# jibo27/3DGS_Hierarchical_Training

Hardware: AMD Instinct MI355X
Metric: train-step images/sec + fwd+bwd ms @1M Gaussians, 980x545; 1/2/4/8 GPU (higher is better)
Workload: dtype f32

## Files before the change

### 3dgs_hierarchical_training_amd/csrc/gsr_kernels.hip

```cpp
#include <hip/hip_runtime.h>
#include <hip/hip_ext.h>
#include <type_traits>
#include <stdint.h>
#include <stdio.h>
#include <string.h>

#include <algorithm>
#include <atomic>
#include <chrono>
#include <cmath>
#include <map>
#include <mutex>
#include <tuple>
#include <vector>

#include "../../include/gsr.h"
#include "gsr_math.h"
#include "adam_math.h"
#include "radix_sort.h"
#include "blend_common.h"

#ifndef GSR_K9_UNROLL
#define GSR_K9_UNROLL 2
#endif
// ... 1080 lines not shown
        for (int g = 0; g < kDbMaxGroups; g++) v[g] = g < db.G ? db.GT[(size_t)g * db.Tp + t] : 0u;
#pragma unroll
        for (int g = 0; g < kDbMaxGroups; g++) {
            if (g < db.G) db.GT[(size_t)g * db.Tp + t] = tot;
            tot += v[g];
        }
    }
    if (t >= db.T) tot = 0u;
    const uint32_t inc = wave_inclusive_sum(tot);
    if (lane == 63) s_w[wave] = inc;
    __syncthreads();
    lo = s_lo[0] + s_lo[1] + s_lo[2] + s_lo[3];
    all = s_all[0] + s_all[1] + s_all[2] + s_all[3];
    uint32_t add = 0u;
#pragma unroll
    for (int w = 0; w < 4; w++) add += w < wave ? s_w[w] : 0u;
    const uint32_t base_t = (uint32_t)min(lo + add + inc - tot, 0xffffffffull);
    if (t < db.T) db.tbase[t] = base_t;
    if (cut.key) {
        if (t < db.T) {
            const uint32_t e = cut.cur[0] < (uint32_t)kVcEntries ? cut.cur[0] : 0u;
            const bool use = cut.cur[9] != 0u && cut.owner_n[e] == (uint32_t)db.N;
            uint32_t ck = (uint32_t)(db.NC - 1);
            const uint32_t k = use ? cut.key[(size_t)e * db.T + t] : kCutOpenKey;
            if (k != kCutOpenKey && k != 0u) {
                const float d = __uint_as_float(k);
                const uint32_t kc = __float_as_uint(fmaf(d, cut.margin, d));
                int a = 0, b = db.NC;
                while (a < b) { const int m = (a + b) >> 1; if (s_bkey[m] <= kc) a = m + 1; else b = m; }
                ck = (uint32_t)max(a - 1, 0);
            }
            cut.chunk[t] = (uint16_t)ck;
            cut.flag[t] = 0u;
            if (use) atomicAdd(&cut.hist[ck], 1u);
            if (t == 0) cut.ctl[3] = use ? 1u : 0u;
        }
    }
    if (slab == 0 && tid == 0) {
        db.tbase[db.T] = (uint32_t)min(all, 0xffffffffull);
        *total_out = all;
        if (host_out) {
            __atomic_store_n(host_out + 2, (unsigned long long)g_onesweep_giveups, __ATOMIC_RELAXED);
            __atomic_store_n(host_out + 3, (unsigned long long)(window_overflow ? *window_overflow : 0u), __ATOMIC_RELAXED);
            __atomic_store_n(host_out, all, __ATOMIC_RELAXED);
            __threadfence_system();
            __atomic_store_n(host_out + 1, host_seq, __ATOMIC_RELAXED);
            __threadfence_system();
        }
        if (late_out) scan_report_late(late_out, all, host_seq);
    }
}

constexpr int kDbPairs = 1024;
__device__ __forceinline__ void lds_order() { __builtin_amdgcn_fence(__ATOMIC_ACQ_REL, "wavefront"); __builtin_amdgcn_wave_barrier(); }

__device__ __forceinline__ uint32_t cut_frame(const ListCut& cut, const int NC, uint32_t& deep)
{
    const int lane = threadIdx.x & 63;
    deep = 0u;
    if (cut.ctl[3] == 0u) return (uint32_t)(NC - 1);
    constexpr int kR = 32;
    uint32_t v[kR];
#pragma unroll
    for (int q = 0; q < kR; q++) { const int c = NC - 1 - 64 * q - lane; v[q] = (64 * q < NC && c >= 0) ? cut.hist[c] : 0u; }
    uint32_t acc = 0u;
#pragma unroll
    for (int q = 0; q < kR; q++) {
        if (64 * q >= NC) break;
        const int c = NC - 1 - 64 * q - lane;
        const uint32_t inc = acc + wave_inclusive_sum(v[q]);
        const unsigned long long over = __ballot(c >= 0 && inc > (uint32_t)cut.dmax);
        if (over) {
            const int l = (int)__builtin_ctzll(over);
            deep = (uint32_t)__builtin_amdgcn_readlane((int)(inc - v[q]), l);
            return (uint32_t)(NC - 1 - 64 * q - l);
        }
        acc = (uint32_t)__builtin_amdgcn_readlane((int)inc, 63);
    }
    for (int top = NC - 1 - 64 * kR; top >= 0; top -= 64) {
        const int c = top - lane;
        const uint32_t w = c >= 0 ? cut.hist[c] : 0u;
        const uint32_t inc = acc + wave_inclusive_sum(w);
        const unsigned long long over = __ballot(c >= 0 && inc > (uint32_t)cut.dmax);
        if (over) {
            const int l = (int)__builtin_ctzll(over);
            deep = (uint32_t)__builtin_amdgcn_readlane((int)(inc - w), l);
            return (uint32_t)(top - l);
        }
        acc = (uint32_t)__builtin_amdgcn_readlane((int)inc, 63);
    }
    deep = acc;
    return 0u;
}

template <typename Want>
__device__ __forceinline__ void cut_chunk_tiles(const DirectBin& db, const int c, const int W, const int H, const int tiles_x, const int tiles_y,
                                                const uint32_t* __restrict__ sorted_gid, const TileRec* __restrict__ sorted_rec,
                                                const Splat* __restrict__ splat, uint32_t* __restrict__ list, const uint32_t cap,
                                                uint32_t* s_txy , uint32_t* s_pos , Want&& want)
{
    const int lane = threadIdx.x & 63;
    const unsigned long long lt = lanemask_lt();
    const int j0 = c * db.S, j1 = min(db.N, j0 + db.S);
    const uint32_t* gt = db.GT + (size_t)(c / db.Cg) * db.Tp;
    const uint16_t* mr = db.M + (size_t)c * db.Tp;
    auto load_rec = [&](int j) -> TileRec { TileRec r; r.mask = 0u; r.rect = 1u << 24; if (j < j1) r = sorted_rec[j]; return r; };
// ... 22 lines not shown
        }
        if (nt == 0) break;
        lds_order();
        TileRec rA = load_rec(j0 + lane), rB = load_rec(j0 + 64 + lane);
        uint32_t gA = load_gid(j0 + lane), gB = load_gid(j0 + 64 + lane);
        for (int j = j0; j < j1; j += 64) {
            const TileRec r = rA;
            const uint32_t g = gA;
            rA = rB; gA = gB;
            rB = load_rec(j + 128 + lane);
            gB = load_gid(j + 128 + lane);
            const bool big = (r.rect & kTileRecBig) != 0u && r.mask != 0u;
            const uint32_t ww = (r.rect >> 24) & 63u, rx0 = r.rect & 0xfffu, ry0 = (r.rect >> 12) & 0xfffu;
            TileTest tt = {};
            int bx0 = 0, by0 = 0, bx1 = 0, by1 = 0;
            if (big) {
                const Splat sp = splat[g];
                tile_rect_tight(sp.px, sp.py, sp.radius, sp.ca, sp.cb, sp.cc, sp.op, W, H, tiles_x, tiles_y, bx0, by0, bx1, by1);
                tt = make_tile_test(sp.px, sp.py, sp.ca, sp.cb, sp.cc, sp.op);
            }
            const bool any_big = __ballot(big) != 0ull;
            for (int k = 0; k < nt; k++) {
                const uint32_t txy = s_txy[k], tx = txy & 0xffffu, ty = txy >> 16;
                const uint32_t dx = tx - rx0, dy = ty - ry0, bit = dy * ww + dx;
                bool in = !big && dx < ww && bit < 32u && ((r.mask >> bit) & 1u) != 0u;
                if (any_big && big) in = (int)tx >= bx0 && (int)tx < bx1 && (int)ty >= by0 && (int)ty < by1 && tile_accept(tt, (int)tx, (int)ty, W, H);
                const unsigned long long b = __ballot(in);
                if (b == 0ull) continue;
                const uint32_t p0 = s_pos[k];
                if (in) { const uint32_t pos = p0 + (uint32_t)__popcll(b & lt); if (pos < cap) list[pos] = g; }
                lds_order();
                if (lane == 0) s_pos[k] = p0 + (uint32_t)__popcll(b);
                lds_order();
            }
        }
        lds_order();
    }
}

#ifdef GSR_DB_TIMING
__device__ unsigned long long g_db_dbg[16];
#define DB_T(k) do { const unsigned long long now_ = __builtin_readcyclecounter(); if (lane == 0) dbt[k] += now_ - dbt_last; dbt_last = now_; } while (0)
#else
#define DB_T(k) do { } while (0)
#endif
template <bool PAIRS = false, int CUT = 0>
__global__ __launch_bounds__(64) void k_chunk_scatter(DirectBin db, int W, int H, int tiles_x, int tiles_y,
                                                      const uint32_t* __restrict__ sorted_gid, const TileRec* __restrict__ sorted_rec,
                                                      const Splat* __restrict__ splat, uint32_t* __restrict__ list, uint2* __restrict__ ranges,
                                                      uint32_t cap, const uint32_t* __restrict__ dkey = nullptr, uint2* __restrict__ pairs = nullptr,
                                                      ListCut cut = ListCut{})
{
    static_assert(!CUT || !PAIRS, "the list cut serves the plain direct binning");
    extern __shared__ unsigned long long s_dyn[];
    const int LT = db.Tp;
    unsigned long long* const s_mask = s_dyn;
    uint32_t* const s_cnt = reinterpret_cast<uint32_t*>(s_dyn + LT);
    uint32_t* const s_pair = s_cnt + LT;
    const int lane = threadIdx.x, b = (int)blockIdx.x;
    if (CUT == 2 && cut.ctl[2] == 0u) return;
    uint32_t cstar = 0u, ndeep = 0u;
    if (CUT == 1) cstar = cut_frame(cut, db.NC, ndeep);
    if (CUT == 2) cstar = cut.ctl[0];
    {
        const int t = b * 64 + lane;
        if (t < db.T) {
            uint32_t tend = db.tbase[t + 1];
            if (CUT == 1) {
                const uint32_t c1 = max((uint32_t)cut.chunk[t], cstar) + 1u;
                if (c1 < (uint32_t)db.NC) tend = db.tbase[t] + db.GT[(size_t)(c1 / (uint32_t)db.Cg) * db.Tp + t] + (uint32_t)db.M[(size_t)c1 * db.Tp + t];
                cut.tend[t] = tend;
            }
            const uint32_t lo = min(db.tbase[t], cap), hi = min(tend, cap);
            if (CUT != 2 || cut.flag[t]) ranges[t] = hi > lo ? make_uint2(lo, hi) : make_uint2(0u, 0u);
            if (CUT == 1) {
                const uint32_t e = cut.cur[0] < (uint32_t)kVcEntries ? cut.cur[0] : 0u;
                cut.key[(size_t)e * db.T + t] = 0u;
            }
        }
        if (CUT && b == 0 && lane == 0) {
            if (CUT == 1) {
                const uint32_t e = cut.cur[0] < (uint32_t)kVcEntries ? cut.cur[0] : 0u;
                cut.owner_n[e] = (uint32_t)db.N;
                cut.ctl[0] = cstar; cut.ctl[1] = ndeep;
                cut.stats[0] += 1u;
                cut.stats[3] += (uint32_t)(db.NC - 1) - min(cstar, (uint32_t)(db.NC - 1));
                cut.stats[4] += ndeep;
            } else { cut.stats[1] += 1u; cut.stats[2] += cut.ctl[2]; }
        }
    }
    const int per = (db.NC + 7) >> 3, kk = b >> 3, c = (b & 7) * per + kk;
    if (kk >= per || c >= db.NC) return;
    if (CUT && (uint32_t)c > cstar) {
        if (CUT == 1 && ndeep == 0u) return;
        uint32_t* const s_tile = s_pair;
        uint32_t* const s_pos = s_pair + 64;
        if (CUT == 1) cut_chunk_tiles(db, c, W, H, tiles_x, tiles_y, sorted_gid, sorted_rec, splat, list, cap, s_tile, s_pos,
                                      [&](uint32_t t) { return (uint32_t)cut.chunk[t] >= (uint32_t)c; });
        else cut_chunk_tiles(db, c, W, H, tiles_x, tiles_y, sorted_gid, sorted_rec, splat, list, cap, s_tile, s_pos,
                             [&](uint32_t t) { return cut.flag[t] != 0u && (uint32_t)cut.chunk[t] < (uint32_t)c; });
        return;
    }
    if (CUT == 2) return;
#ifdef GSR_DB_TIMING
    unsigned long long dbt[8] = {0, 0, 0, 0, 0, 0, 0, 0}, dbt_last = __builtin_readcyclecounter();
#endif
    {
        const uint32_t* gt = db.GT + (size_t)(c / db.Cg) * db.Tp;
        const uint16_t* mr = db.M + (size_t)c * db.Tp;
        constexpr int kRows = 36;
        for (int i0 = 0; i0 < LT; i0 += 64 * kRows) {
            uint32_t tb[kRows], gb[kRows], mc[kRows];
#pragma unroll
            for (int q = 0; q < kRows; q++) {
                const int i = i0 + 64 * q + lane;
                const bool v = i < LT && (uint32_t)i < (uint32_t)LT;
                tb[q] = v && i < db.T ? db.tbase[i] : 0u;
                gb[q] = v ? gt[i] : 0u;
                mc[q] = v ? (uint32_t)mr[i] : 0u;
            }
#pragma unroll
            for (int q = 0; q < kRows; q++) {
                const int i = i0 + 64 * q + lane;
                if (i < LT) { s_cnt[i] = tb[q] + gb[q] + mc[q]; s_mask[i] = 0ull; }
            }
        }
    }
    lds_order();
    DB_T(0);
    const unsigned long long me = 1ull << lane, lt = lanemask_lt();
    const int j0 = c * db.S, j1 = min(db.N, j0 + db.S);
    auto load_gid = [&](int j) -> uint32_t { return j < j1 ? (PAIRS ? (uint32_t)j : sorted_gid[j]) : 0u; };
    auto load_rec = [&](int j) -> TileRec { TileRec r; r.mask = 0u; r.rect = 1u << 24; if (j < j1) r = sorted_rec[j]; return r; };
    auto load_key = [&](int j) -> uint32_t { return (PAIRS && j < j1) ? dkey[j] : 0u; };
    uint32_t gA = load_gid(j0 + lane), gB = load_gid(j0 + 64 + lane);
    TileRec rA = load_rec(j0 + lane), rB = load_rec(j0 + 64 + lane);
    uint32_t kA = load_key(j0 + lane), kB = load_key(j0 + 64 + lane);
    for (int j = j0 + lane; j - lane < j1; j += 64) {
        const uint32_t g = gA;
        TileRec r = rA;
        const uint32_t kd = kA;
        gA = gB; rA = rB; kA = kB;
        gB = load_gid(j + 128);
        rB = load_rec(j + 128);
        kB = load_key(j + 128);
        const bool big = (r.rect & kTileRecBig) != 0u && r.mask != 0u, huge = big && r.mask > (uint32_t)kDbPairs;
        const unsigned long long bigs = __ballot(big && !huge), huges = __ballot(huge);
        const uint32_t cnt = huge ? 0u : tilerec_count(r);
        const uint32_t incl = wave_inclusive_sum(cnt);
        auto run_end = [&](int lo, uint32_t before) -> int {
            const unsigned long long over = __ballot(incl - before > (uint32_t)kDbPairs) & ~((1ull << lo) - 1ull);
            return over ? (int)__builtin_ctzll(over) : 64;
        };
        auto owners = [&](int lo, int hi, uint32_t before, bool with_or) {
            const bool mine = lane >= lo && lane < hi;
            if (!big && (with_or || mine)) {
                uint32_t* o = s_pair + (incl - cnt - before);
                small_rect_tiles(r, tiles_x, [&](uint32_t t) {
                    if (with_or) atomicOr(&s_mask[t], me);
                    if (mine) *o++ = (t << 6) | (uint32_t)lane;
                });
            }
            for (unsigned long long bm = bigs; bm != 0ull; bm &= bm - 1ull) {
                const int bl = (int)__builtin_ctzll(bm);
                const bool in_run = bl >= lo && bl < hi;
                if (!with_or && !in_run) continue;
                const uint32_t gg = (uint32_t)__builtin_amdgcn_readlane((int)g, bl), rect = (uint32_t)__builtin_amdgcn_readlane((int)r.rect, bl);
                uint32_t o = (uint32_t)__builtin_amdgcn_readlane((int)(incl - cnt), bl) - before;
                const Splat s = splat[gg];
                big_rect_tiles(s, rect, W, H, tiles_x, tiles_y, lane, [&](bool ok, uint32_t t) {
                    const unsigned long long acc = __ballot(ok);
                    if (ok) {
                        if (with_or) atomicOr(&s_mask[t], 1ull << bl);
                        if (in_run) s_pair[(o + (uint32_t)__popcll(acc & lt)) & (uint32_t)(kDbPairs - 1)] = (t << 6) | (uint32_t)bl;
                    }
                    o += (uint32_t)__popcll(acc);
                });
            }
        };
        int lo = 0, hi = run_end(0, 0u);
        uint32_t before = 0u;
        const bool one_run = hi == 64;
        DB_T(1);
        owners(0, hi, 0u, true);
        DB_T(2);
        for (unsigned long long bm = huges; bm != 0ull; bm &= bm - 1ull) {
            const int bl = (int)__builtin_ctzll(bm);
            const uint32_t gg = (uint32_t)__builtin_amdgcn_readlane((int)g, bl), rect = (uint32_t)__builtin_amdgcn_readlane((int)r.rect, bl);
            const Splat s = splat[gg];
            big_rect_tiles(s, rect, W, H, tiles_x, tiles_y, lane, [&](bool ok, uint32_t t) { if (ok && t < (uint32_t)db.T) atomicOr(&s_mask[t], 1ull << bl); });
        }
        asm volatile("" : "+v"(gA), "+v"(rA.mask), "+v"(rA.rect));
        if (PAIRS) asm volatile("" : "+v"(kA));
        lds_order();
        DB_T(3);
        for (;;) {
            const uint32_t P = (uint32_t)__builtin_amdgcn_readlane((int)incl, hi - 1) - before;
            for (uint32_t p0 = 0u; p0 < P; p0 += 512u) {
                const uint32_t left = P - p0;
                auto batch = [&](auto rounds_tag) {
                    constexpr int RN = decltype(rounds_tag)::value;
                    uint32_t e[RN], go[RN], base[RN], ko[PAIRS ? RN : 1];
                    unsigned long long mk[RN];
#pragma unroll
                    for (int q = 0; q < RN; q++) e[q] = s_pair[(p0 + 64u * q + (uint32_t)lane) & (uint32_t)(kDbPairs - 1)];
#pragma unroll
                    for (int q = 0; q < RN; q++) {
                        const bool v = 64u * q + (uint32_t)lane < left;
                        e[q] = v ? e[q] : 0xffffffffu;
                        const uint32_t t = v ? e[q] >> 6 : 0u;
                        go[q] = (uint32_t)__builtin_amdgcn_ds_bpermute((int)((e[q] & 63u) << 2), (int)g);
                        if (PAIRS) ko[q] = (uint32_t)__builtin_amdgcn_ds_bpermute((int)((e[q] & 63u) << 2), (int)kd);
                        mk[q] = s_mask[t];
                        base[q] = s_cnt[t];
                    }
#pragma unroll
                    for (int q = 0; q < RN; q++)
                        if (e[q] != 0xffffffffu) {
                            const uint32_t pos = base[q] + (uint32_t)__popcll(mk[q] & ((1ull << (e[q] & 63u)) - 1ull));
                            if (pos < cap) {
                                if (PAIRS) pairs[pos] = make_uint2(ko[q], go[q]);
                                else list[pos] = go[q];
                            }
                        }
                };
                if (left <= 128u) batch(std::integral_constant<int, 2>{});
                else if (left <= 256u) batch(std::integral_constant<int, 4>{});
                else if (left <= 384u) batch(std::integral_constant<int, 6>{});
                else batch(std::integral_constant<int, 8>{});
            }
            if (hi == 64) break;
            lds_order();
            before += P;
            lo = hi;
            hi = run_end(lo, before);
            owners(lo, hi, before, false);
            lds_order();
        }
        for (unsigned long long bm = huges; bm != 0ull; bm &= bm - 1ull) {
            const int bl = (int)__builtin_ctzll(bm);
            const uint32_t gg = (uint32_t)__builtin_amdgcn_readlane((int)g, bl), rect = (uint32_t)__builtin_amdgcn_readlane((int)r.rect, bl);
            const Splat s = splat[gg];
            big_rect_tiles(s, rect, W, H, tiles_x, tiles_y, lane, [&](bool ok, uint32_t t) {
                if (ok && t < (uint32_t)db.T) {
                    const uint32_t pos = s_cnt[t] + (uint32_t)__popcll(s_mask[t] & ((1ull << bl) - 1ull));
                    if (pos < cap) {
                        if (PAIRS) pairs[pos] = make_uint2((uint32_t)__builtin_amdgcn_readlane((int)kd, bl), gg);
                        else list[pos] = gg;
                    }
                }
            });
        }
        lds_order();
        DB_T(4);
        if (one_run) {
            const uint32_t P = (uint32_t)__builtin_amdgcn_readlane((int)incl, 63);
            for (uint32_t p0 = 0u; p0 < P; p0 += 512u) {
                const uint32_t left = P - p0;
                auto batch = [&](auto rounds_tag) {
                    constexpr int RN = decltype(rounds_tag)::value;
                    uint32_t e[RN];
#pragma unroll
                    for (int q = 0; q < RN; q++) e[q] = s_pair[(p0 + 64u * q + (uint32_t)lane) & (uint32_t)(kDbPairs - 1)];
#pragma unroll
                    for (int q = 0; q < RN; q++)
                        if (64u * q + (uint32_t)lane < left) { atomicAdd(&s_cnt[e[q] >> 6], 1u); s_mask[e[q] >> 6] = 0ull; }
                };
                if (left <= 128u) batch(std::integral_constant<int, 2>{});
                else if (left <= 256u) batch(std::integral_constant<int, 4>{});
                else if (left <= 384u) batch(std::integral_constant<int, 6>{});
                else batch(std::integral_constant<int, 8>{});
            }
        } else {
            if (!big) small_rect_tiles(r, tiles_x, [&](uint32_t t) { atomicAdd(&s_cnt[t], 1u); s_mask[t] = 0ull; });
            for (unsigned long long bm = bigs; bm != 0ull; bm &= bm - 1ull) {
                const int bl = (int)__builtin_ctzll(bm);
                const uint32_t gg = (uint32_t)__builtin_amdgcn_readlane((int)g, bl), rect = (uint32_t)__builtin_amdgcn_readlane((int)r.rect, bl);
                const Splat s = splat[gg];
                big_rect_tiles(s, rect, W, H, tiles_x, tiles_y, lane, [&](bool ok, uint32_t t) { if (ok && t < (uint32_t)db.T) { atomicAdd(&s_cnt[t], 1u); s_mask[t] = 0ull; } });
            }
        }
        for (unsigned long long bm = huges; bm != 0ull; bm &= bm - 1ull) {
            const int bl = (int)__builtin_ctzll(bm);
            const uint32_t gg = (uint32_t)__builtin_amdgcn_readlane((int)g, bl), rect = (uint32_t)__builtin_amdgcn_readlane((int)r.rect, bl);
            const Splat s = splat[gg];
            big_rect_tiles(s, rect, W, H, tiles_x, tiles_y, lane, [&](bool ok, uint32_t t) { if (ok && t < (uint32_t)db.T) { atomicAdd(&s_cnt[t], 1u); s_mask[t] = 0ull; } });
        }
        lds_order();
        DB_T(5);
    }
#ifdef GSR_DB_TIMING
    if (lane == 0) {
        for (int k = 0; k < 6; k++) atomicAdd(&g_db_dbg[k], dbt[k]);
        atomicAdd(&g_db_dbg[6], 1ull);
        atomicAdd(&g_db_dbg[7], (unsigned long long)((j1 - j0 + 63) / 64));
    }
#endif
}

constexpr int kTsCap = 4096, kTsSmallMax = 1024;

template <int THREADS, int IPT, bool GATHER = false>
__device__ __forceinline__ void tile_sort_regs(const uint2* __restrict__ src, uint32_t* dst, uint32_t n, const uint32_t* __restrict__ dkey,
                                               unsigned long long (*s_mask)[256], uint32_t (*s_cnt)[256], uint32_t* s_keys, uint32_t* s_vals,
                                               uint32_t* s_start, uint32_t* s_wsum, uint32_t* s_bits)
{
    constexpr int WAVES = THREADS / 64;
    const int tid = threadIdx.x, wave = tid >> 6, lane = tid & 63;
    uint32_t key[IPT], val[IPT], dig[IPT], rnk[IPT];
    uint32_t k_or = 0u, k_and = 0xffffffffu;
#pragma unroll
    for (int r = 0; r < IPT; r++) {
        const uint32_t p = (uint32_t)(wave * (IPT * 64) + r * 64 + lane);
        if (GATHER) val[r] = p < n ? dst[p] : 0u;
        else if (p < n) { const uint2 e = src[p]; key[r] = e.x; val[r] = e.y; }
        if (!GATHER && p >= n) { key[r] = 0xffffffffu; val[r] = 0u; }
    }
    if (GATHER) {
#pragma unroll
        for (int r = 0; r < IPT; r++) {
            const uint32_t p = (uint32_t)(wave * (IPT * 64) + r * 64 + lane);
            key[r] = p < n ? dkey[val[r]] : 0xffffffffu;
        }
    }
#pragma unroll
    for (int r = 0; r < IPT; r++) {
        const uint32_t p = (uint32_t)(wave * (IPT * 64) + r * 64 + lane);
        if (p < n) { k_or |= key[r]; k_and &= key[r]; }
    }
#pragma unroll
    for (int off = 32; off > 0; off >>= 1) { k_or |= (uint32_t)__shfl_xor((int)k_or, off, 64); k_and &= (uint32_t)__shfl_xor((int)k_and, off, 64); }
    if (lane == 0) { s_bits[wave] = k_or; s_bits[WAVES + wave] = k_and; }
    __syncthreads();
    uint32_t differ = 0u;
    {
        uint32_t o = 0u, a = 0xffffffffu;
#pragma unroll
        for (int w = 0; w < WAVES; w++) { o |= s_bits[w]; a &= s_bits[WAVES + w]; }
        differ = o & ~a;
    }
#pragma unroll 1
    for (int shift = 0; shift < 32; shift += 8) {
        if (((differ >> shift) & 0xffu) == 0u) continue;
#pragma unroll
        for (int r = 0; r < IPT; r++) dig[r] = (key[r] >> shift) & 0xffu;
        wave_rank<IPT, 256>(s_mask[wave], s_cnt[wave], dig, rnk, lane);
// ... 2260 lines not shown
        if (hipGetDevice(&dev_id) != hipSuccess || hipDeviceSynchronize() != hipSuccess) return GSR_ERR_HIP;
        std::lock_guard<std::mutex> lk(g_state_mutex);
        for (auto& c : g_view_costs)
            if (c.dev == dev_id && hipMemset(c.mem, 0, c.bytes) != hipSuccess) return GSR_ERR_HIP;
        return GSR_OK;
    }
    if (!strcmp(name, "list_cut_margin_e3")) { g_list_cut_margin_e3 = value < 0 ? 50 : value; return GSR_OK; }
    if (!strcmp(name, "list_cut_deep")) { g_list_cut_deep = value < 0 ? 8 : value; return GSR_OK; }
    if (!strcmp(name, "debug_late_bias")) { g_debug_late_bias = value; return GSR_OK; }
    if (!strcmp(name, "tile_sort")) { if (value < 0 || value > 2) return GSR_ERR_ARG; g_tile_sort = value; return GSR_OK; }
    if (!strcmp(name, "tile_sort_max_avg")) { if (value < 0) return GSR_ERR_ARG; g_tile_sort_max_avg = value; return GSR_OK; }
    if (!strcmp(name, "view_pose_tol_e6")) { if (value < 0) return GSR_ERR_ARG; g_view_pose_tol_e6 = value; return GSR_OK; }
    if (!strcmp(name, "depth_sort9")) { g_depth_sort9 = value ? 1 : 0; return GSR_OK; }
    if (!strcmp(name, "direct_binning")) { g_direct_bin = value ? 1 : 0; return GSR_OK; }
    if (!strcmp(name, "speculative_binning")) { g_speculate = value ? 1 : 0; return GSR_OK; }
    if (!strcmp(name, "deterministic_backward")) { g_deterministic = value ? 1 : 0; return GSR_OK; }
    if (!strcmp(name, "binning_capacity_hint")) {
        std::lock_guard<std::mutex> lk(g_state_mutex);
        g_hint_override = value > 0 ? value : -1;
        return GSR_OK;
    }
    if (!strcmp(name, "reset_speculation")) {
        std::lock_guard<std::mutex> lk(g_state_mutex);
        g_hints.clear(); g_hint_override = -1;
        g_spec_overflows = 0; g_spec_forwards = 0; g_exact_forwards = 0; g_depth_window_resorts = 0;
        g_full_depth_sort.clear();
        return GSR_OK;
    }
    if (!strcmp(name, "profile")) { g_profile = (value == 2 || value == 3) ? value : (value ? 1 : 0); g_profile_tick = 0; return GSR_OK; }
    if (!strcmp(name, "prep_hist_max_n")) { g_prep_hist_max_n = value; return GSR_OK; }
    if (!strcmp(name, "small_sort9")) { if (value < 0) return GSR_ERR_ARG; g_small_sort9 = value; return GSR_OK; }
    if (!strcmp(name, "poll_iters")) { g_poll_iters = value < 0 ? 0 : value; return GSR_OK; }
    if (!strcmp(name, "emit_hist")) { g_emit_hist = value ? 1 : 0; return GSR_OK; }
    if (!strcmp(name, "sort_algo")) { if (value < 0 || value > 2) return GSR_ERR_ARG; g_sort_algo = value; return GSR_OK; }
    if (!strcmp(name, "blend_bwd_ppt")) {
        if (value < 0 || value > 2) return GSR_ERR_ARG;
        g_bwd_ppt = value; return GSR_OK;
    }
    return GSR_ERR_ARG;
}

struct DirectBinScratch { size_t M, GT, tbase, bsum, cut_chunk, cut_tend, cut_flag, cut_ctl, cut_bkey, cut_hist, bytes; };
static bool direct_bin_geometry(int N, int T, DirectBin& db, DirectBinScratch& ds)
{
    if (N < 1 || T < 1 || T > kDbMaxTiles) return false;
    static std::atomic<int> cus_cached{0};
    int cus = cus_cached.load(std::memory_order_relaxed);
    if (!cus) {
        int dev = 0, n = 0;
        cus = (hipGetDevice(&dev) == hipSuccess && hipDeviceGetAttribute(&n, hipDeviceAttributeMultiprocessorCount, dev) == hipSuccess && n > 0) ? n : 256;
        cus_cached.store(cus, std::memory_order_relaxed);
    }
    db.N = N; db.T = T; db.Tp = (T + 63) & ~63;
    const int lds = 12 * db.Tp + 4 * kDbPairs;
    const int per_cu = std::min(16, (160 * 1024) / lds);
    const long long resident = std::max<long long>(1, (long long)cus * per_cu);
    const int min_s = 128;
    long long S = ((long long)N + resident - 1) / resident;
    S = std::max<long long>(min_s, (S + 63) & ~63ll);
    if (S > 65472) return false;
    db.S = (int)S;
    db.NC = (int)(((long long)N + S - 1) / S);
    int G = 1;
    while (G * G < db.NC) G++;
    db.Cg = std::max(1, std::min((db.NC + G - 1) / G, 65535 / db.S));
    db.G = (db.NC + db.Cg - 1) / db.Cg;
    if (db.G > kDbMaxGroups) return false;
    size_t o = 0;
    ds.M = o; o += align256((size_t)db.NC * db.Tp * sizeof(uint16_t));
    ds.GT = o; o += align256((size_t)db.G * db.Tp * sizeof(uint32_t));
    ds.tbase = o; o += align256((size_t)(db.Tp + 1) * sizeof(uint32_t));
    ds.bsum = o; o += align256((size_t)db.G * ((db.Tp + 255) / 256) * sizeof(uint32_t));
    ds.cut_chunk = o; o += align256((size_t)db.Tp * sizeof(uint16_t));
    ds.cut_tend = o; o += align256((size_t)db.Tp * sizeof(uint32_t));
    ds.cut_flag = o; o += align256((size_t)db.Tp * sizeof(uint32_t));
    ds.cut_ctl = o; o += 256;
    ds.cut_bkey = o; o += align256((size_t)db.NC * sizeof(uint32_t));
    ds.cut_hist = o; o += align256((size_t)db.NC * sizeof(uint32_t));
    ds.bytes = o;
    return true;
}

int gsr_forward(const GsrForwardArgs* a, GsrForwardOut* out, void* stream_)
{
    CallTimer call_timer(g_fwd_calls, g_fwd_ns);
    hipStream_t st = (hipStream_t)stream_;
    if (!a || !out) return fail(GSR_ERR_ARG, "null args%s");
    int rc = check_common(a->N, a->M, a->D, a->W, a->H);
    if (rc) return rc;
    if (!a->out_color || !a->out_depth || !a->out_alpha || !a->image || !a->bg || !a->alloc)
        return fail(GSR_ERR_ARG, "missing output / workspace pointer%s");
    const int N = a->N, W = a->W, H = a->H;
    BatchDev bt;
    rc = batch_dev(a->batch, N, H, bt);
    if (rc) return rc;
    const int NB = bt.B;
    const int opt_ppt = g_blend_ppt ? g_blend_ppt : 7, opt_map = g_tile_map, opt_ckpt = g_ckpt_first;
    const int tiles_x = (W + kTile - 1) / kTile, tiles_y = (H + kTile - 1) / kTile, T = tiles_x * tiles_y * NB;
    if (a->sh_origin && (!a->shs || NB > 1 || a->prepared))
        return fail(GSR_ERR_ARG, "sh_origin needs shs and is not served with a batch of B > 1 or a prepared buffer%s");
    out->num_rendered = 0; out->binning = nullptr; out->binning_bytes = 0; out->binning_capacity = 0;
    out->forward_flags = pack_fwd_flags(opt_ppt, opt_map, opt_ckpt);
    uint64_t R = 0;
    BlendBalance bb = {};
    ListCut lc = {};
    uint64_t lc_capacity = 0;
    Splat* splat = static_cast<Splat*>(a->geom);
    float* img = static_cast<float*>(a->image);
// ... 42 lines not shown
    auto launch_binning_t = [&](auto key_tag, uint64_t capacity, const unsigned long long* n_dev, bool prezeroed) -> int {
        using KeyT = decltype(key_tag);
        if (!prezeroed) GSR_HIP(hipMemsetAsync(ranges, 0, (size_t)T * sizeof(uint2), st));
        if (capacity == 0) return GSR_OK;
        KeyT* tkey = reinterpret_cast<KeyT*>(bs + S.tile);
        KeyT* tkey_alt = reinterpret_cast<KeyT*>(bs + S.tile_alt);
        uint32_t* gid_alt2 = reinterpret_cast<uint32_t*>(bs + S.gid_alt);
        uint32_t* block_sums = reinterpret_cast<uint32_t*>(fs + L.block_sums);
        uint32_t* v0 = (tile_passes & 1) ? gid_alt2 : list;
        uint32_t* v1 = (tile_passes & 1) ? list : gid_alt2;
        const bool emit_hist = g_sort_algo == 2 && prezeroed && g_emit_hist;
        EmitHist eh = {};
        if (emit_hist) {
            eh.ghist = reinterpret_cast<uint32_t*>(bs + S.sort);
            eh.status = onesweep_status(bs + S.sort);
            eh.status_words = onesweep_status_words<KeyT>((uint32_t)capacity, bits);
            eh.bits = bits;
            eh.n_dev = n_dev;
        }
        {
            ProfScope ps(P_EMIT, st);
            hipLaunchKernelGGL(k_emit<KeyT>, dim3(nb), dim3(kEmitThreads), 0, st, N, W, H, tiles_x, tiles_y, sorted_gid, splat,
                               tsort ? ts_rec : reinterpret_cast<const TileRec*>(fs + L.srec), block_sums, tkey, v0,
                               (uint32_t)capacity, eh);
        }
        int in_alt = 0;
        {
            ProfScope ps(P_SORT_TILE, st);
            GSR_HIP(g_sort_algo == 2 ? onesweep_sort_pairs<KeyT>(tkey, v0, tkey_alt, v1, (uint32_t)capacity, 0, bits, bs + S.sort,
                                                                 &in_alt, st, n_dev, prezeroed, emit_hist)
                                     : radix_sort_pairs<KeyT>(tkey, v0, tkey_alt, v1, (uint32_t)capacity, 0, tile_passes * 8, bs + S.sort,
                                                              &in_alt, st));
        }
        const KeyT* skey = in_alt ? tkey_alt : tkey;
        {
            ProfScope ps(P_RANGES, st);
            constexpr uint32_t kpb = 256u * (16u / (uint32_t)sizeof(KeyT));
            hipLaunchKernelGGL(k_tile_ranges<KeyT>, dim3(((uint32_t)capacity + kpb - 1) / kpb), dim3(256), 0, st, (uint32_t)capacity, skey, ranges, n_dev);
        }
        if (tsort) {
            ProfScope ps(P_SORT_DEPTH, st);
            hipLaunchKernelGGL(k_tile_sort_wave<true>, dim3(T), dim3(64), 0, st, ranges, pairs, list, T, ts_dkey);
            hipLaunchKernelGGL((k_tile_sort<1024, true>), dim3(std::min(T, 512)), dim3(1024), 0, st, ranges, pairs, pairs_alt, list, T, ts_dkey);
        }
        return GSR_OK;
    };
    auto launch_binning = [&](uint64_t capacity, const unsigned long long* n_dev, bool prezeroed) -> int {
        if (direct) {
            if (capacity == 0) { GSR_HIP(hipMemsetAsync(ranges, 0, (size_t)T * sizeof(uint2), st)); return GSR_OK; }
            const int per = (db.NC + 7) / 8, grid = std::max(8 * per, (T + 63) / 64);
            if (tsort) {
                {
                    ProfScope ps(P_EMIT, st);
                    hipLaunchKernelGGL((k_chunk_scatter<true>), dim3(grid), dim3(64), (size_t)12 * db.Tp + 4 * kDbPairs, st, db, W, H, tiles_x, tiles_y,
                                       (const uint32_t*)nullptr, ts_rec, splat, list, ranges, (uint32_t)std::min<uint64_t>(capacity, 0xffffffffull), ts_dkey, pairs);
                }
                ProfScope ps2(P_SORT_TILE, st);
                hipLaunchKernelGGL(k_tile_sort_wave<false>, dim3(T), dim3(64), 0, st, ranges, pairs, list, T, (const uint32_t*)nullptr);
                hipLaunchKernelGGL(k_tile_sort<1024>, dim3(std::min(T, 512)), dim3(1024), 0, st, ranges, pairs, pairs_alt, list, T);
                return GSR_OK;
            }
            ProfScope ps(P_EMIT, st);
            if (lc.key) {
                lc_capacity = capacity;
                hipLaunchKernelGGL((k_chunk_scatter<false, 1>), dim3(grid), dim3(64), (size_t)12 * db.Tp + 4 * kDbPairs, st, db, W, H,
                                   tiles_x, tiles_y, sorted_gid, reinterpret_cast<const TileRec*>(fs + L.srec), splat, list, ranges,
                                   (uint32_t)std::min<uint64_t>(capacity, 0xffffffffull), (const uint32_t*)nullptr, (uint2*)nullptr, lc);
            } else
                hipLaunchKernelGGL(k_chunk_scatter<false>, dim3(grid), dim3(64), (size_t)12 * db.Tp + 4 * kDbPairs, st, db, W, H, tiles_x, tiles_y, sorted_gid,
                                   reinterpret_cast<const TileRec*>(fs + L.srec), splat, list, ranges, (uint32_t)std::min<uint64_t>(capacity, 0xffffffffull));
            return GSR_OK;
        }
        return wide_keys ? launch_binning_t(uint32_t{}, capacity, n_dev, prezeroed) : launch_binning_t(uint16_t{}, capacity, n_dev, prezeroed);
    };
    auto launch_blend = [&](bool prezeroed) -> int {
        const int ppt = opt_ppt;
        if (!prezeroed) GSR_HIP(hipMemsetAsync(staged, 0, (size_t)T * 16, st));
        float* ckpt = reinterpret_cast<float*>(bin + B.ckpt);
        if (ppt == 7 && g_profile && (g_profile != 3 || g_profile_tick.fetch_add(1u) % 3u == 0u)) {
            hipEvent_t ea = nullptr, eb = nullptr;
            if (hipEventCreate(&ea) != hipSuccess || hipEventCreate(&eb) != hipSuccess) return fail(GSR_ERR_HIP, "hipEventCreate failed%s");
            hipExtLaunchKernelGGL(k_blend_fwd_w6<true>, dim3(8 * 4 * slots_per_xcd(opt_map, T, tiles_x)), dim3(64), 0, st, ea, eb, 0, W, H, tiles_x, T, ranges, list,
                                  splat, a->bg, a->out_color, a->out_depth, a->out_alpha, img, staged, opt_map, ckpt, opt_ckpt, tiles_y, bb, a->out_color_clamped,
                                  lc, lc.key ? 1 : 0);
            std::lock_guard<std::mutex> lk(g_prof_mutex);
            g_prof_events[P_BLEND_FWD].push_back({ea, eb});
        } else {
            ProfScope ps(ppt == 7 && g_profile == 3 ? P_COUNT : P_BLEND_FWD, st);
            if (ppt == 7)
                hipLaunchKernelGGL(k_blend_fwd_w6<true>, dim3(8 * 4 * slots_per_xcd(opt_map, T, tiles_x)), dim3(64), 0, st, W, H, tiles_x, T, ranges, list, splat, a->bg,
                                   a->out_color, a->out_depth, a->out_alpha, img, staged, opt_map, ckpt, opt_ckpt, tiles_y, bb, a->out_color_clamped,
                                   lc, lc.key ? 1 : 0);
            else
                hipLaunchKernelGGL(k_blend_fwd_w6<false>, dim3(8 * 4 * slots_per_xcd(opt_map, T, tiles_x)), dim3(64), 0, st, W, H, tiles_x, T, ranges, list, splat, a->bg,
                                   a->out_color, a->out_depth, a->out_alpha, img, staged, opt_map, ckpt, opt_ckpt, tiles_y, BlendBalance{}, a->out_color_clamped);
        }
        if (ppt == 7 && lc.key && lc_capacity > 0) {
            ProfScope ps(P_CUT_REPAIR, st);
            const int per = (db.NC + 7) / 8, grid = std::max(8 * per, (T + 63) / 64);
            hipLaunchKernelGGL((k_chunk_scatter<false, 2>), dim3(grid), dim3(64), (size_t)12 * db.Tp + 4 * kDbPairs, st, db, W, H,
                               tiles_x, tiles_y, sorted_gid, reinterpret_cast<const TileRec*>(fs + L.srec), splat, list, ranges,
                               (uint32_t)std::min<uint64_t>(lc_capacity, 0xffffffffull), (const uint32_t*)nullptr, (uint2*)nullptr, lc);
            hipLaunchKernelGGL(k_blend_fwd_w6<true>, dim3(8 * 4 * slots_per_xcd(opt_map, T, tiles_x)), dim3(64), 0, st, W, H, tiles_x, T, ranges, list, splat, a->bg,
                               a->out_color, a->out_depth, a->out_alpha, img, staged, opt_map, ckpt, opt_ckpt, tiles_y, bb, a->out_color_clamped, lc, 2);
        }
        GSR_HIP(hipGetLastError());
        return GSR_OK;
    };

    if (N == 0) {
        rc = alloc_binning(0);
        if (rc) return rc;
        rc = launch_binning(0, nullptr, false);
        if (rc) return rc;
        rc = launch_blend(false);
        if (rc) return rc;
        out->binning = bin;
        out->binning_bytes = B.bytes;
        return GSR_OK;
    }

    if (!a->means3D || !a->opacities || !a->geom || !a->radii || !a->viewmatrix || !a->projmatrix)
        return fail(GSR_ERR_ARG, "missing input pointer%s");
    if ((a->shs == nullptr) == (a->colors_precomp == nullptr)) return fail(GSR_ERR_ARG, "provide exactly one of shs / colors_precomp%s");
    if ((a->cov3D_precomp == nullptr) == (a->scales == nullptr || a->rotations == nullptr))
        return fail(GSR_ERR_ARG, "provide exactly one of (scales, rotations) / cov3D_precomp%s");
    if (a->shs && (!a->campos || a->M < (a->D + 1) * (a->D + 1))) return fail(GSR_ERR_ARG, "shs needs campos and M >= (D+1)^2%s");

    int dev_id = 0;
    GSR_HIP(hipGetDevice(&dev_id));
    const auto hint_key = std::make_tuple(dev_id, W, H * NB, n_bucket(N));
    uint64_t hint = 0;
    {
        std::lock_guard<std::mutex> lk(g_state_mutex);
        if (g_hint_override > 0) { hint = (uint64_t)g_hint_override; g_hint_override = -1; }
        else { auto it = g_hints.find(hint_key); if (it != g_hints.end()) hint = it->second; }
    }
    const bool speculative = g_speculate && g_sort_algo == 2 && hint > 0;
    const uint64_t cap = speculative ? hint : 0;
    {
        const int ts_mode = g_tile_sort;
        const uint64_t avg = (hint > 0 ? hint : (uint64_t)N * 4u) / (uint64_t)T;
        const bool auto_ok = ts_mode == 1 && avg <= (uint64_t)g_tile_sort_max_avg && (direct || N / std::max(1, NB) <= g_tile_sort_emit_max_n);
        tsort = (ts_mode == 2 || auto_ok) && g_sort_algo == 2 && (direct ? NB == 1 : true);
    }

    fs = static_cast<uint8_t*>(a->alloc(align256(L.bytes) + (direct ? dbs.bytes : 0), GSR_ALLOC_SCRATCH, a->alloc_user));
    if (!fs) return fail(GSR_ERR_ALLOC, "scratch allocation failed%s");
    if (speculative) {
        rc = alloc_binning(cap);
        if (rc) return rc;
    }
    uint32_t* dkey = reinterpret_cast<uint32_t*>(fs + L.dkey);
// ... 700 lines not shown
```

Measured before the change: 1203.

## Replace per-tile lane bitmasks with LDS atomic counters in chunk scatter

The direct-binning scatter kernel drops the per-tile 64-bit lane mask (atomicOr pass plus popcount rank) and instead claims positions with LDS atomicAdd on the per-tile counter. Intra-wave collisions on the same tile are ranked with ballot/readlane, huge splats are handled inline as separate runs, and the post-pass that advanced counters and cleared masks is removed. This cuts the LDS footprint from 12 to 4 bytes per tile, which allows more resident waves, and removes several passes over tile rects. The cost is atomic contention and extra ballot loops when many lanes hit the same tile. Output order within a tile may change if the atomics do not preserve lane order.

Result: no change. 1209, median of 4 (+0.5%).

```diff
diff --git a/3dgs_hierarchical_training_amd/csrc/gsr_kernels.hip b/3dgs_hierarchical_training_amd/csrc/gsr_kernels.hip
--- a/3dgs_hierarchical_training_amd/csrc/gsr_kernels.hip
+++ b/3dgs_hierarchical_training_amd/csrc/gsr_kernels.hip
@@ -1156,6 +1156,8 @@
 }
 
 constexpr int kDbPairs = 1024;
+constexpr int direct_bin_lds(int Tp) { return 4 * Tp + 4 * kDbPairs; }
+constexpr int kDbWavesPerCu = 16;
 __device__ __forceinline__ void lds_order() { __builtin_amdgcn_fence(__ATOMIC_ACQ_REL, "wavefront"); __builtin_amdgcn_wave_barrier(); }
 
 __device__ __forceinline__ uint32_t cut_frame(const ListCut& cut, const int NC, uint32_t& deep)
@@ -1284,10 +1286,9 @@
                                                       ListCut cut = ListCut{})
 {
     static_assert(!CUT || !PAIRS, "the list cut serves the plain direct binning");
-    extern __shared__ unsigned long long s_dyn[];
+    extern __shared__ uint32_t s_dyn[];
     const int LT = db.Tp;
-    unsigned long long* const s_mask = s_dyn;
-    uint32_t* const s_cnt = reinterpret_cast<uint32_t*>(s_dyn + LT);
+    uint32_t* const s_cnt = s_dyn;
     uint32_t* const s_pair = s_cnt + LT;
     const int lane = threadIdx.x, b = (int)blockIdx.x;
     if (CUT == 2 && cut.ctl[2] == 0u) return;
@@ -1354,7 +1355,7 @@
 #pragma unroll
             for (int q = 0; q < kRows; q++) {
                 const int i = i0 + 64 * q + lane;
-                if (i < LT) { s_cnt[i] = tb[q] + gb[q] + mc[q]; s_mask[i] = 0ull; }
+                if (i < LT) s_cnt[i] = tb[q] + gb[q] + mc[q];
             }
         }
     }
@@ -1381,80 +1382,82 @@
         const uint32_t cnt = huge ? 0u : tilerec_count(r);
         const uint32_t incl = wave_inclusive_sum(cnt);
         auto run_end = [&](int lo, uint32_t before) -> int {
-            const unsigned long long over = __ballot(incl - before > (uint32_t)kDbPairs) & ~((1ull << lo) - 1ull);
+            const unsigned long long over = (__ballot(incl - before > (uint32_t)kDbPairs) | huges) & ~((1ull << lo) - 1ull);
             return over ? (int)__builtin_ctzll(over) : 64;
         };
-        auto owners = [&](int lo, int hi, uint32_t before, bool with_or) {
-            const bool mine = lane >= lo && lane < hi;
-            if (!big && (with_or || mine)) {
+        auto owners = [&](int lo, int hi, uint32_t before) {
+            if (!big && lane >= lo && lane < hi) {
                 uint32_t* o = s_pair + (incl - cnt - before);
-                small_rect_tiles(r, tiles_x, [&](uint32_t t) {
-                    if (with_or) atomicOr(&s_mask[t], me);
-                    if (mine) *o++ = (t << 6) | (uint32_t)lane;
-                });
+                small_rect_tiles(r, tiles_x, [&](uint32_t t) { *o++ = (t << 6) | (uint32_t)lane; });
             }
             for (unsigned long long bm = bigs; bm != 0ull; bm &= bm - 1ull) {
                 const int bl = (int)__builtin_ctzll(bm);
-                const bool in_run = bl >= lo && bl < hi;
-                if (!with_or && !in_run) continue;
+                if (bl < lo || bl >= hi) continue;
                 const uint32_t gg = (uint32_t)__builtin_amdgcn_readlane((int)g, bl), rect = (uint32_t)__builtin_amdgcn_readlane((int)r.rect, bl);
                 uint32_t o = (uint32_t)__builtin_amdgcn_readlane((int)(incl - cnt), bl) - before;
                 const Splat s = splat[gg];
                 big_rect_tiles(s, rect, W, H, tiles_x, tiles_y, lane, [&](bool ok, uint32_t t) {
                     const unsigned long long acc = __ballot(ok);
-                    if (ok) {
-                        if (with_or) atomicOr(&s_mask[t], 1ull << bl);
-                        if (in_run) s_pair[(o + (uint32_t)__popcll(acc & lt)) & (uint32_t)(kDbPairs - 1)] = (t << 6) | (uint32_t)bl;
-                    }
+                    if (ok) s_pair[(o + (uint32_t)__popcll(acc & lt)) & (uint32_t)(kDbPairs - 1)] = (t << 6) | (uint32_t)bl;
                     o += (uint32_t)__popcll(acc);
                 });
             }
         };
         int lo = 0, hi = run_end(0, 0u);
         uint32_t before = 0u;
-        const bool one_run = hi == 64;
         DB_T(1);
-        owners(0, hi, 0u, true);
+        owners(0, hi, 0u);
         DB_T(2);
-        for (unsigned long long bm = huges; bm != 0ull; bm &= bm - 1ull) {
-            const int bl = (int)__builtin_ctzll(bm);
-            const uint32_t gg = (uint32_t)__builtin_amdgcn_readlane((int)g, bl), rect = (uint32_t)__builtin_amdgcn_readlane((int)r.rect, bl);
-            const Splat s = splat[gg];
-            big_rect_tiles(s, rect, W, H, tiles_x, tiles_y, lane, [&](bool ok, uint32_t t) { if (ok && t < (uint32_t)db.T) atomicOr(&s_mask[t], 1ull << bl); });
-        }
         asm volatile("" : "+v"(gA), "+v"(rA.mask), "+v"(rA.rect));
         if (PAIRS) asm volatile("" : "+v"(kA));
         lds_order();
         DB_T(3);
         for (;;) {
-            const uint32_t P = (uint32_t)__builtin_amdgcn_readlane((int)incl, hi - 1) - before;
+            const uint32_t P = hi > lo ? (uint32_t)__builtin_amdgcn_readlane((int)incl, hi - 1) - before : 0u;
             for (uint32_t p0 = 0u; p0 < P; p0 += 512u) {
                 const uint32_t left = P - p0;
                 auto batch = [&](auto rounds_tag) {
                     constexpr int RN = decltype(rounds_tag)::value;
-                    uint32_t e[RN], go[RN], base[RN], ko[PAIRS ? RN : 1];
-                    unsigned long long mk[RN];
+                    uint32_t e[RN], go[RN], b0[RN], b1[RN], ko[PAIRS ? RN : 1];
 #pragma unroll
                     for (int q = 0; q < RN; q++) e[q] = s_pair[(p0 + 64u * q + (uint32_t)lane) & (uint32_t)(kDbPairs - 1)];
 #pragma unroll
                     for (int q = 0; q < RN; q++) {
-                        const bool v = 64u * q + (uint32_t)lane < left;
-                        e[q] = v ? e[q] : 0xffffffffu;
-                        const uint32_t t = v ? e[q] >> 6 : 0u;
+                        e[q] = 64u * q + (uint32_t)lane < left ? e[q] : 0xffffffffu;
                         go[q] = (uint32_t)__builtin_amdgcn_ds_bpermute((int)((e[q] & 63u) << 2), (int)g);
                         if (PAIRS) ko[q] = (uint32_t)__builtin_amdgcn_ds_bpermute((int)((e[q] & 63u) << 2), (int)kd);
-                        mk[q] = s_mask[t];
-                        base[q] = s_cnt[t];
                     }
 #pragma unroll
-                    for (int q = 0; q < RN; q++)
+                    for (int q = 0; q < RN; q++) {
+                        b0[q] = 0u; b1[q] = 1u;
                         if (e[q] != 0xffffffffu) {
-                            const uint32_t pos = base[q] + (uint32_t)__popcll(mk[q] & ((1ull << (e[q] & 63u)) - 1ull));
+                            volatile uint32_t* const ctr = &s_cnt[e[q] >> 6];
+                            b0[q] = *ctr;
+                            lds_order();
+                            atomicAdd(&s_cnt[e[q] >> 6], 1u);
+                            lds_order();
+                            b1[q] = *ctr;
+                        }
+                        lds_order();
+                    }
+#pragma unroll
+                    for (int q = 0; q < RN; q++) {
+                        const uint32_t t = e[q] >> 6;
+                        uint32_t rk = 0u;
+                        for (unsigned long long shared = __ballot(b1[q] - b0[q] != 1u); shared != 0ull;) {
+                            const uint32_t tt = (uint32_t)__builtin_amdgcn_readlane((int)t, (int)__builtin_ctzll(shared));
+                            const unsigned long long peers = __ballot(t == tt);
+                            if (t == tt) rk = (uint32_t)__popcll(peers & lt);
+                            shared &= ~peers;
+                        }
+                        if (e[q] != 0xffffffffu) {
+                            const uint32_t pos = b0[q] + rk;
                             if (pos < cap) {
                                 if (PAIRS) pairs[pos] = make_uint2(ko[q], go[q]);
                                 else list[pos] = go[q];
                             }
                         }
+                    }
                 };
                 if (left <= 128u) batch(std::integral_constant<int, 2>{});
                 else if (left <= 256u) batch(std::integral_constant<int, 4>{});
@@ -1464,66 +1467,33 @@
             if (hi == 64) break;
             lds_order();
             before += P;
+            if ((huges >> hi) & 1ull) {
+                const uint32_t gg = (uint32_t)__builtin_amdgcn_readlane((int)g, hi), rect = (uint32_t)__builtin_amdgcn_readlane((int)r.rect, hi);
+                const uint32_t kk2 = PAIRS ? (uint32_t)__builtin_amdgcn_readlane((int)kd, hi) : 0u;
+                const Splat s = splat[gg];
+                big_rect_tiles(s, rect, W, H, tiles_x, tiles_y, lane, [&](bool ok, uint32_t t) {
+                    if (ok && t < (uint32_t)db.T) {
+                        const uint32_t pos = atomicAdd(&s_cnt[t], 1u);
+                        if (pos < cap) {
+                            if (PAIRS) pairs[pos] = make_uint2(kk2, gg);
+                            else list[pos] = gg;
+                        }
+                    }
+                });
+                lds_order();
+                if (++hi == 64) break;
+            }
             lo = hi;
             hi = run_end(lo, before);
-            owners(lo, hi, before, false);
+            owners(lo, hi, before);
             lds_order();
-        }
-        for (unsigned long long bm = huges; bm != 0ull; bm &= bm - 1ull) {
-            const int bl = (int)__builtin_ctzll(bm);
-            const uint32_t gg = (uint32_t)__builtin_amdgcn_readlane((int)g, bl), rect = (uint32_t)__builtin_amdgcn_readlane((int)r.rect, bl);
-            const Splat s = splat[gg];
-            big_rect_tiles(s, rect, W, H, tiles_x, tiles_y, lane, [&](bool ok, uint32_t t) {
-                if (ok && t < (uint32_t)db.T) {
-                    const uint32_t pos = s_cnt[t] + (uint32_t)__popcll(s_mask[t] & ((1ull << bl) - 1ull));
-                    if (pos < cap) {
-                        if (PAIRS) pairs[pos] = make_uint2((uint32_t)__builtin_amdgcn_readlane((int)kd, bl), gg);
-                        else list[pos] = gg;
-                    }
-                }
-            });
         }
         lds_order();
         DB_T(4);
-        if (one_run) {
-            const uint32_t P = (uint32_t)__builtin_amdgcn_readlane((int)incl, 63);
-            for (uint32_t p0 = 0u; p0 < P; p0 += 512u) {
-                const uint32_t left = P - p0;
-                auto batch = [&](auto rounds_tag) {
-                    constexpr int RN = decltype(rounds_tag)::value;
-                    uint32_t e[RN];
-#pragma unroll
-                    for (int q = 0; q < RN; q++) e[q] = s_pair[(p0 + 64u * q + (uint32_t)lane) & (uint32_t)(kDbPairs - 1)];
-#pragma unroll
-                    for (int q = 0; q < RN; q++)
-                        if (64u * q + (uint32_t)lane < left) { atomicAdd(&s_cnt[e[q] >> 6], 1u); s_mask[e[q] >> 6] = 0ull; }
-                };
-                if (left <= 128u) batch(std::integral_constant<int, 2>{});
-                else if (left <= 256u) batch(std::integral_constant<int, 4>{});
-                else if (left <= 384u) batch(std::integral_constant<int, 6>{});
-                else batch(std::integral_constant<int, 8>{});
-            }
-        } else {
-            if (!big) small_rect_tiles(r, tiles_x, [&](uint32_t t) { atomicAdd(&s_cnt[t], 1u); s_mask[t] = 0ull; });
-            for (unsigned long long bm = bigs; bm != 0ull; bm &= bm - 1ull) {
-                const int bl = (int)__builtin_ctzll(bm);
-                const uint32_t gg = (uint32_t)__builtin_amdgcn_readlane((int)g, bl), rect = (uint32_t)__builtin_amdgcn_readlane((int)r.rect, bl);
-                const Splat s = splat[gg];
-                big_rect_tiles(s, rect, W, H, tiles_x, tiles_y, lane, [&](bool ok, uint32_t t) { if (ok && t < (uint32_t)db.T) { atomicAdd(&s_cnt[t], 1u); s_mask[t] = 0ull; } });
-            }
-        }
-        for (unsigned long long bm = huges; bm != 0ull; bm &= bm - 1ull) {
-            const int bl = (int)__builtin_ctzll(bm);
-            const uint32_t gg = (uint32_t)__builtin_amdgcn_readlane((int)g, bl), rect = (uint32_t)__builtin_amdgcn_readlane((int)r.rect, bl);
-            const Splat s = splat[gg];
-            big_rect_tiles(s, rect, W, H, tiles_x, tiles_y, lane, [&](bool ok, uint32_t t) { if (ok && t < (uint32_t)db.T) { atomicAdd(&s_cnt[t], 1u); s_mask[t] = 0ull; } });
-        }
-        lds_order();
-        DB_T(5);
     }
 #ifdef GSR_DB_TIMING
     if (lane == 0) {
-        for (int k = 0; k < 6; k++) atomicAdd(&g_db_dbg[k], dbt[k]);
+        for (int k = 0; k < 5; k++) atomicAdd(&g_db_dbg[k], dbt[k]);
         atomicAdd(&g_db_dbg[6], 1ull);
         atomicAdd(&g_db_dbg[7], (unsigned long long)((j1 - j0 + 63) / 64));
     }
@@ -3890,8 +3860,8 @@
         cus_cached.store(cus, std::memory_order_relaxed);
     }
     db.N = N; db.T = T; db.Tp = (T + 63) & ~63;
-    const int lds = 12 * db.Tp + 4 * kDbPairs;
-    const int per_cu = std::min(16, (160 * 1024) / lds);
+    const int lds = direct_bin_lds(db.Tp);
+    const int per_cu = std::min(kDbWavesPerCu, (160 * 1024) / lds);
     const long long resident = std::max<long long>(1, (long long)cus * per_cu);
     const int min_s = 128;
     long long S = ((long long)N + resident - 1) / resident;
@@ -4040,7 +4010,7 @@
             if (tsort) {
                 {
                     ProfScope ps(P_EMIT, st);
-                    hipLaunchKernelGGL((k_chunk_scatter<true>), dim3(grid), dim3(64), (size_t)12 * db.Tp + 4 * kDbPairs, st, db, W, H, tiles_x, tiles_y,
+                    hipLaunchKernelGGL((k_chunk_scatter<true>), dim3(grid), dim3(64), (size_t)direct_bin_lds(db.Tp), st, db, W, H, tiles_x, tiles_y,
                                        (const uint32_t*)nullptr, ts_rec, splat, list, ranges, (uint32_t)std::min<uint64_t>(capacity, 0xffffffffull), ts_dkey, pairs);
                 }
                 ProfScope ps2(P_SORT_TILE, st);
@@ -4051,11 +4021,11 @@
             ProfScope ps(P_EMIT, st);
             if (lc.key) {
                 lc_capacity = capacity;
-                hipLaunchKernelGGL((k_chunk_scatter<false, 1>), dim3(grid), dim3(64), (size_t)12 * db.Tp + 4 * kDbPairs, st, db, W, H,
+                hipLaunchKernelGGL((k_chunk_scatter<false, 1>), dim3(grid), dim3(64), (size_t)direct_bin_lds(db.Tp), st, db, W, H,
                                    tiles_x, tiles_y, sorted_gid, reinterpret_cast<const TileRec*>(fs + L.srec), splat, list, ranges,
                                    (uint32_t)std::min<uint64_t>(capacity, 0xffffffffull), (const uint32_t*)nullptr, (uint2*)nullptr, lc);
             } else
-                hipLaunchKernelGGL(k_chunk_scatter<false>, dim3(grid), dim3(64), (size_t)12 * db.Tp + 4 * kDbPairs, st, db, W, H, tiles_x, tiles_y, sorted_gid,
+                hipLaunchKernelGGL(k_chunk_scatter<false>, dim3(grid), dim3(64), (size_t)direct_bin_lds(db.Tp), st, db, W, H, tiles_x, tiles_y, sorted_gid,
                                    reinterpret_cast<const TileRec*>(fs + L.srec), splat, list, ranges, (uint32_t)std::min<uint64_t>(capacity, 0xffffffffull));
             return GSR_OK;
         }
@@ -4086,7 +4056,7 @@
         if (ppt == 7 && lc.key && lc_capacity > 0) {
             ProfScope ps(P_CUT_REPAIR, st);
             const int per = (db.NC + 7) / 8, grid = std::max(8 * per, (T + 63) / 64);
-            hipLaunchKernelGGL((k_chunk_scatter<false, 2>), dim3(grid), dim3(64), (size_t)12 * db.Tp + 4 * kDbPairs, st, db, W, H,
+            hipLaunchKernelGGL((k_chunk_scatter<false, 2>), dim3(grid), dim3(64), (size_t)direct_bin_lds(db.Tp), st, db, W, H,
                                tiles_x, tiles_y, sorted_gid, reinterpret_cast<const TileRec*>(fs + L.srec), splat, list, ranges,
                                (uint32_t)std::min<uint64_t>(lc_capacity, 0xffffffffull), (const uint32_t*)nullptr, (uint2*)nullptr, lc);
             hipLaunchKernelGGL(k_blend_fwd_w6<true>, dim3(8 * 4 * slots_per_xcd(opt_map, T, tiles_x)), dim3(64), 0, st, W, H, tiles_x, T, ranges, list, splat, a->bg,
```
